# debarghabhattofficial/yolo_tracking

Hardware: AMD Instinct MI355X
Metric: tracker.update() calls/sec @ 1024 tracks×1024 dets; 1/2/4/8 MI355X (higher is better)
Workload: dtype f64; 1 GPU; bytetrack 1024x1024, 2048 streams/GPU, inputs resident in HBM; tracker=bytetrack, tracks=1024, dets=1024, streams_per_gpu=2048, queues_per_gpu=2, parallelism=stream-sharded x1, preroll=35

## Files before the change

include/yolo_tracking_amd.h:

```cpp
#ifndef YOLO_TRACKING_AMD_H
#define YOLO_TRACKING_AMD_H

#include <stdint.h>

#ifdef __cplusplus
extern "C" {
#endif

#define YTA_OK 0
#define YTA_ERR_INVALID (-1)
#define YTA_ERR_HIP (-2)
#define YTA_ERR_CAPACITY (-3)
#define YTA_ERR_NOMEM (-4)

int yta_version(void);
const char *yta_last_error(void);
int yta_device_count(int *count);

#define YTA_AFF_IOU 0
#define YTA_AFF_GIOU 1
#define YTA_AFF_DIOU 2
#define YTA_AFF_CIOU 3
#define YTA_AFF_CENTROID 4
int yta_box_affinity(int device, int kind, const double *a, int na, const double *b, int nb,
                     double img_w, double img_h, double *out);
int yta_iou_distance(int device, const double *a, int na, const double *b, int nb,
                     const double *scores, double *out);

int yta_grid_pairs(int device, const double *a, int na, const double *b, int nb, double thresh,
                   int *pairs, int cap, int *n_pairs);

int yta_kf_xyah_initiate(int device, int n, const double *meas, double *mean, double *cov);
int yta_affine_apply(int device, int kind, int n, const double *warps, double *mean, double *cov);
int yta_kf_xyah_predict(int device, int n, double *mean, double *cov);
int yta_kf_xyah_update(int device, int n, double *mean, double *cov, const double *z);

int yta_selftest(int device);

int yta_apply_block_map(int gx, int n_streams, int *stream, int *block);

int yta_lap_limited(int device, int nr, int nc, const double *cost, double cost_limit, int *x,
                    int *y);

int yta_lap_padded(int device, int nr, int nc, const double *cost, int *x, int *y);

int yta_lap_rect(int device, int nr, int nc, const double *cost, int *x, int *y);
int yta_lap_first_round(int device, int na, int nb, const double *cost, int *rx, int *done,
                        int *n_tight);

typedef struct yta_bytetrack yta_bytetrack;
typedef struct {
    double track_thresh;
    double match_thresh;
    int track_buffer;
    int frame_rate;
} yta_bytetrack_params;

int yta_bytetrack_create(int device, int n_streams, int track_capacity, int max_dets,
                         const yta_bytetrack_params *params, yta_bytetrack **engine);
int yta_bytetrack_destroy(yta_bytetrack *engine);
int yta_bytetrack_reset(yta_bytetrack *engine);

int yta_bytetrack_reserve(yta_bytetrack *engine, int track_capacity, int max_dets);
int yta_bytetrack_capacity(yta_bytetrack *engine, int *track_capacity, int *max_dets);

int yta_bytetrack_update(yta_bytetrack *engine, const double *dets, const int *det_offsets,
                         long long *next_id, double *out, int out_capacity, int *out_offsets);

int yta_bytetrack_update_device(yta_bytetrack *engine, const double *d_dets,
                                const int *d_det_offsets, double *d_out, int *d_out_counts);
int yta_bytetrack_sync(yta_bytetrack *engine);
int yta_bytetrack_next_ids(yta_bytetrack *engine, long long *next_id);

int yta_bytetrack_submit(yta_bytetrack *engine, const double *dets, const int *det_offsets,
                         const long long *next_id, double *out, int out_capacity);
int yta_bytetrack_collect(yta_bytetrack *engine, long long *next_id, int *out_offsets);
int yta_bytetrack_pipe_stats(yta_bytetrack *engine, double *stats, int n, int reset);
int yta_bytetrack_submit_f32(yta_bytetrack *engine, const float *dets, const int *det_offsets,
                             const long long *next_id, double *out, int out_capacity);
int yta_bytetrack_update_f32(yta_bytetrack *engine, const float *dets, const int *det_offsets,
                             long long *next_id, double *out, int out_capacity,
                             int *out_offsets);

int yta_bytetrack_update_streams(yta_bytetrack *engine, int n_streams, const int *stream_ids,
                                 const double *dets, const int *det_offsets, long long *next_id,
                                 double *out, int out_capacity, int *out_offsets);
int yta_bytetrack_update_device_masked(yta_bytetrack *engine, const int *d_active,
                                       const double *d_dets, const int *d_det_offsets,
                                       double *d_out, int *d_out_counts);
int yta_bytetrack_reset_stream(yta_bytetrack *engine, int stream);

int yta_bytetrack_get_state(yta_bytetrack *engine, int stream, int *n_tracks, long long *ints,
// ... 314 lines not shown
```

yolo_tracking_amd/_lib.py:

```python
import ctypes
import os

import numpy as np

_HERE = os.path.dirname(os.path.abspath(__file__))
LIB_PATH = os.environ.get("YTA_LIBRARY") or os.path.join(_HERE, "libyta.so")


class PwArgs(ctypes.Structure):
    _fields_ = [("x1", ctypes.c_void_p), ("x1n", ctypes.c_longlong), ("x1c", ctypes.c_longlong),
                ("x1p", ctypes.c_longlong), ("x2", ctypes.c_void_p), ("x2n", ctypes.c_longlong),
                ("x2c", ctypes.c_longlong), ("x2p", ctypes.c_longlong), ("w", ctypes.c_void_p),
                ("bias", ctypes.c_void_p), ("res", ctypes.c_void_p), ("rn", ctypes.c_longlong),
                ("rc", ctypes.c_longlong), ("rp", ctypes.c_longlong), ("y", ctypes.c_void_p),
                ("yn", ctypes.c_longlong), ("yc", ctypes.c_longlong), ("yp", ctypes.c_longlong),
                ("k1", ctypes.c_int), ("k2", ctypes.c_int), ("G", ctypes.c_int),
                ("cout_g", ctypes.c_int), ("P", ctypes.c_int), ("N", ctypes.c_int),
                ("relu", ctypes.c_int), ("pad", ctypes.c_int)]


YTA_OK = 0
YTA_ERR_INVALID = -1
YTA_ERR_HIP = -2
YTA_ERR_CAPACITY = -3
# ... 68 lines not shown
    "yta_device_count": ([_P], _I),
    "yta_box_affinity": ([_I, _I, _P, _I, _P, _I, _D, _D, _P], _I),
    "yta_iou_distance": ([_I, _P, _I, _P, _I, _P, _P], _I),
    "yta_kf_xyah_initiate": ([_I, _I, _P, _P, _P], _I),
    "yta_kf_xyah_predict": ([_I, _I, _P, _P], _I),
    "yta_kf_xyah_update": ([_I, _I, _P, _P, _P], _I),
    "yta_grid_pairs": ([_I, _P, _I, _P, _I, _D, _P, _I, _P], _I),
    "yta_lap_limited": ([_I, _I, _I, _P, _D, _P, _P], _I),
    "yta_lap_padded": ([_I, _I, _I, _P, _P, _P], _I),
    "yta_lap_rect": ([_I, _I, _I, _P, _P, _P], _I),
    "yta_lap_first_round": ([_I, _I, _I, _P, _P, _P, _P], _I),
    "yta_affine_apply": ([_I, _I, _I, _P, _P, _P], _I),
    "yta_bytetrack_create": ([_I, _I, _I, _I, _P, _P], _I),
    "yta_bytetrack_destroy": ([_P], _I),
    "yta_bytetrack_reset": ([_P], _I),
    "yta_bytetrack_reserve": ([_P, _I, _I], _I),
    "yta_bytetrack_capacity": ([_P, _P, _P], _I),
    "yta_bytetrack_update": ([_P, _P, _P, _P, _P, _I, _P], _I),
    "yta_bytetrack_update_device": ([_P, _P, _P, _P, _P], _I),
    "yta_bytetrack_sync": ([_P], _I),
    "yta_bytetrack_update_streams": ([_P, _I, _P, _P, _P, _P, _P, _I, _P], _I),
    "yta_bytetrack_update_device_masked": ([_P, _P, _P, _P, _P, _P], _I),
    "yta_bytetrack_reset_stream": ([_P, _I], _I),
    "yta_bytetrack_submit": ([_P, _P, _P, _P, _P, _I], _I),
    "yta_bytetrack_collect": ([_P, _P, _P], _I),
    "yta_bytetrack_pipe_stats": ([_P, _P, _I, _I], _I),
    "yta_bytetrack_next_ids": ([_P, _P], _I),
    "yta_bytetrack_submit_f32": ([_P, _P, _P, _P, _P, _I], _I),
    "yta_bytetrack_update_f32": ([_P, _P, _P, _P, _P, _I, _P], _I),
    "yta_bytetrack_get_state": ([_P, _I, _P, _P, _P, _P], _I),
    "yta_bytetrack_profile": ([_P, _I], _I),
    "yta_bytetrack_profile_collect": ([_P, _P, _P], _I),
    "yta_bytetrack_stats": ([_P, _P], _I),
    "yta_bytetrack_modes": ([_P, _P, _I], _I),
    "yta_bytetrack_hip_stream": ([_P, _P], _I),
    "yta_bytetrack_set_lds": ([_P, _I], _I),
    "yta_bytetrack_update_tensors": ([_P, _P, _P, _I, _LL, _P, _P, _P, _P, _LL, _P, _P], _I),
    "yta_bytetrack_tensor_stats": ([_P, _P, _I], _I),
    "yta_botsort_update_tensors": ([_P, _P, _P, _I, _LL, _P, _P, _LL, _P, _P, _P, _P, _LL, _P, _P],
                                   _I),
    "yta_ocsort_update_tensors": ([_P, _P, _P, _I, _LL, _P, _P, _P, _P, _P, _LL, _P, _P], _I),
    "yta_ocsort_tensor_stats": ([_P, _P, _I], _I),
    "yta_ocsort_next_ids": ([_P, _P], _I),
    "yta_deepocsort_update_tensors": ([_P, _P, _P, _I, _LL, _P, _P, _LL, _P, _P, _P, _P, _P, _LL,
                                       _P, _P], _I),
    "yta_deepocsort_tensor_stats": ([_P, _P, _I], _I),
    "yta_deepocsort_next_ids": ([_P, _P], _I),
    "yta_hybridsort_update_tensors": ([_P, _P, _P, _I, _LL, _P, _P, _LL, _P, _P, _P, _LL, _P, _P],
                                      _I),
    "yta_hybridsort_tensor_stats": ([_P, _P, _I], _I),
    "yta_hybridsort_next_ids": ([_P, _P], _I),
    "yta_selftest": ([_I], _I),
    "yta_apply_block_map": ([_I, _I, _P, _P], _I),
    "yta_botsort_create": ([_I, _I, _I, _I, _I, _P, _P], _I),
    "yta_botsort_update": ([_P, _P, _P, _P, _P, _P, _P, _I, _P], _I),
    "yta_botsort_update_device": ([_P, _P, _P, _P, _P, _P, _P], _I),
    "yta_botsort_get_features": ([_P, _I, _P, _P, _P, _P], _I),
    "yta_botsort_update_streams": ([_P, _I, _P, _P, _P, _P, _P, _P, _P, _I, _P], _I),
    "yta_ocsort_create": ([_I, _I, _I, _I, _P, _P], _I),
    "yta_ocsort_destroy": ([_P], _I),
    "yta_ocsort_reset": ([_P], _I),
    "yta_ocsort_capacity": ([_P, _P, _P], _I),
    "yta_ocsort_update": ([_P, _P, _P, _P, _P, _P, _I, _P], _I),
    "yta_ocsort_update_device": ([_P, _P, _P, _P, _P, _P], _I),
    "yta_ocsort_update_streams": ([_P, _I, _P, _P, _P, _P, _P, _P, _I, _P], _I),
    "yta_ocsort_update_device_masked": ([_P, _P, _P, _P, _P, _P, _P], _I),
    "yta_ocsort_reset_stream": ([_P, _I], _I),
    "yta_ocsort_sync": ([_P], _I),
    "yta_ocsort_get_state": ([_P, _I, _P, _P, _P, _P], _I),
    "yta_ocsort_stats": ([_P, _P], _I),
    "yta_ocsort_lap_stats": ([_P, _P, _I], _I),
    "yta_ocsort_hip_stream": ([_P, _P], _I),
    "yta_kf7_run": ([_I, _I, _I, _P, _P, _P, _P], _I),
    "yta_deepocsort_create": ([_I, _I, _I, _I, _I, _P, _P], _I),
    "yta_deepocsort_destroy": ([_P], _I),
    "yta_deepocsort_reset": ([_P], _I),
    "yta_deepocsort_capacity": ([_P, _P, _P], _I),
    "yta_deepocsort_update": ([_P, _P, _P, _P, _P, _P, _P, _P, _I, _P], _I),
    "yta_deepocsort_update_device": ([_P, _P, _P, _P, _P, _P, _P, _P], _I),
    "yta_deepocsort_update_streams": ([_P, _I, _P, _P, _P, _P, _P, _P, _P, _P, _I, _P], _I),
    "yta_deepocsort_update_device_masked": ([_P, _P, _P, _P, _P, _P, _P, _P, _P], _I),
    "yta_deepocsort_reset_stream": ([_P, _I], _I),
    "yta_deepocsort_sync": ([_P], _I),
    "yta_deepocsort_get_state": ([_P, _I, _P, _P, _P, _P, _P], _I),
    "yta_deepocsort_stats": ([_P, _P], _I),
    "yta_deepocsort_lap_stats": ([_P, _P, _I], _I),
    "yta_deepocsort_hip_stream": ([_P, _P], _I),
    "yta_kf8_run": ([_I, _I, _I, _P, _P, _P, _P, _P], _I),
    "yta_hybridsort_create": ([_I, _I, _I, _I, _I, _P, _P], _I),
    "yta_hybridsort_destroy": ([_P], _I),
    "yta_hybridsort_reset": ([_P], _I),
    "yta_hybridsort_capacity": ([_P, _P, _P], _I),
    "yta_hybridsort_update": ([_P, _P, _P, _P, _P, _P, _I, _P], _I),
    "yta_hybridsort_update_device": ([_P, _P, _P, _P, _P, _P], _I),
    "yta_hybridsort_update_streams": ([_P, _I, _P, _P, _P, _P, _P, _P, _I, _P], _I),
    "yta_hybridsort_update_device_masked": ([_P, _P, _P, _P, _P, _P, _P], _I),
    "yta_hybridsort_reset_stream": ([_P, _I], _I),
    "yta_hybridsort_sync": ([_P], _I),
    "yta_hybridsort_get_state": ([_P, _I, _P, _P, _P, _P, _P, _P], _I),
    "yta_hybridsort_classes": ([_P, _I, _P, _I, _P], _I),
    "yta_hybridsort_stats": ([_P, _P], _I),
    "yta_hybridsort_lap_stats": ([_P, _P, _I], _I),
    "yta_hybridsort_hip_stream": ([_P, _P], _I),
    "yta_kf9_run": ([_I, _I, _I, _P, _P, _P, _P], _I),
    "yta_gsi_interpolate": ([_I, _P, _I, _I, _I, _I, _P, ctypes.c_longlong, _P], _I),
    "yta_gsi_smooth": ([_I, _P, _P, _P, _P, _P, _I, _P], _I),
# ... 255 lines not shown
```

yolo_tracking_amd/csrc/bytetrack.hip:

```cpp
#include <chrono>
#include <algorithm>
#include <cmath>
#include <cstring>
#include <memory>
#include <new>
#include <thread>
#include <vector>

#include "bytetrack.hpp"
#include "host_pool.hpp"
#include "oc_host.hpp"

namespace yta {
namespace {

#ifndef YTA_BLK1
#define YTA_BLK1 1024
#endif
#ifndef YTA_BLK23
#define YTA_BLK23 256
#endif
#ifndef YTA_BLKF
#define YTA_BLKF 256
#endif
// ... 586 lines not shown
        const bool give = nd <= 2 * nt && 5LL * 8 * nh <= hand_cap;
        handed = give;
#pragma unroll
        for (int h = 0; h < 2; ++h) {
            const int e = h ? t0 + e1 : e0;
            if (cat[h] == 1) {
                const int p = n_high + (e & 0xFFFF);
                a.high[db + p] = h ? i1 : i0;
                a.high_box[db + p] = b[h];
                a.high_score[db + p] = r[h].v[4];
                if (give) {
                    hand[p] = b[h].x1;
                    hand[nh + p] = b[h].y1;
                    hand[2 * nh + p] = b[h].x2;
                    hand[3 * nh + p] = b[h].y2;
                    hand[4 * nh + p] = r[h].v[4];
                }
            } else if (cat[h] == 2) {
                const int p = n_second + (e >> 16);
                a.second[db + p] = h ? i1 : i0;
                a.second_box[db + p] = b[h];
            }
        }
        n_high += nh;
        n_second += ns;
    }
    s1_frame_counters(a.cnt + s, nd, n_high, n_second);
    return n_high;
}

template <typename F>
__device__ __forceinline__ void s1_row_edges(const BtArgs &a, int s, const GridView &gv,
                                             const GridHdr &h, const Box &rb, F f) {
    const long long db = (long long)s * a.MAXD;
    const double thresh = a.match_thresh;
    auto scored = [&](int j, const Box &cb, double w) {
        const double dist = 1 - iou(rb, cb);
        const double cost = 1 - (1 - dist) * w;
        if (cost < thresh) f(j, cost);
    };
    grid_query(gv, h, rb, scored, [&](int j) {
        const Box cb = a.high_box[db + j];
        if (intersects(rb, cb)) scored(j, cb, a.high_score[db + j]);
    });
}

__device__ __forceinline__ GridView s1_grid_hbm(const BtArgs &a, int s) {
    const long long db = (long long)s * a.MAXD;
    return GridView{a.g_hdr + s, a.g_cell + (long long)s * (GRID_MAX_CELLS + 1), a.g_ids + db,
                    a.g_boxes + db, a.g_w + db, a.g_big + db};
}

__host__ __device__ inline long long s1_grid_bytes(long long C) {
    return 4 * (GRID_MAX_CELLS + 1) + C * (4 + 32 + 8 + 4) + 5 * 16;
}

template <typename HBox, typename HW>
__device__ __forceinline__ void s1_edges_body(const BtArgs &a, int s, int nc, int nr,
                                              const GridView &gv, HBox hbox, HW hw,
                                              GridScratch &gs, int *wsum, int &spill, int *cdeg,
                                              int &n_edges, int (&rn)[4], int (&rc)[4]) {
    const int t = threadIdx.x, nt = blockDim.x;
    const long long tb = (long long)s * a.CAP, SC = (long long)a.S * a.CAP;
    grid_build(nc, hbox, hw, gv, gs, wsum);
    const GridHdr h = gs.hdr;
    YTA_STAMP(1);
    for (int base = t; base < nr; base += 4 * nt) {
        Box rb[4];
#pragma unroll
        for (int b = 0; b < 4; ++b)
            if (base + b * nt < nr) rb[b] = a.pool_box[tb + base + b * nt];
#pragma unroll
        for (int b = 0; b < 4; ++b) {
            const int i = base + b * nt;
            if (i >= nr) continue;
            int n = 0, first = -1;
            s1_row_edges(a, s, gv, h, rb[b], [&](int j, double cost) {
                if (n == 0) first = j;
                if (n < E_SLOTS) {
                    a.e_col[n * SC + tb + i] = j;
                    a.e_cost[n * SC + tb + i] = cost;
                }
                ++n;
                atomicAdd(cdeg + j, 1);
            });
            a.e_cnt[tb + i] = n;
            if (n > E_SLOTS) spill = 1;
            if (n) atomicAdd(&n_edges, n);
            if (base == t) {
                rn[b] = n;
                rc[b] = n == 1 ? first : -1;
            }
        }
    }
}

constexpr int WQ_CAP = 384;
__device__ __forceinline__ Box s1_box(const GridView &gv, int k) {
    const double *x = gv.sx;
    const int n = gv.sn;
    return Box{x[k], x[n + k], x[2 * n + k], x[3 * n + k]};
}
struct EdgeWaveQ {
    unsigned q[WQ_CAP];
    int cnt[WAVE];
    int first[WAVE];
};

__device__ __forceinline__ double bperm_f64(double v, int src_lane) {
    const long long b = __double_as_longlong(v);
    const int lo = __builtin_amdgcn_ds_bpermute(src_lane << 2, (int)b);
    const int hi = __builtin_amdgcn_ds_bpermute(src_lane << 2, (int)(b >> 32));
    return __longlong_as_double(((long long)hi << 32) | (unsigned)lo);
}

__device__ __forceinline__ void s1_edges_rows_wave(const BtArgs &a, int s, int nr,
                                                   const GridView &gv, const GridHdr &h,
                                                   EdgeWaveQ &wq, int &spill, int *cdeg,
                                                   int &n_edges, int (&rn)[4], int (&rc)[4]) {
    const int t = threadIdx.x, nt = blockDim.x, lane = lane_id();
    const long long tb = (long long)s * a.CAP, db = (long long)s * a.MAXD;
    const long long SC = (long long)a.S * a.CAP;
    const double thresh = a.match_thresh;
    int m = 0;
    for (int base = t - lane; base < nr; base += nt, ++m) {
        const int i = base + lane;
        const bool on = i < nr;
        Box rb{0.0, 0.0, 0.0, 0.0};
        if (on) rb = a.pool_box[tb + i];
        int cx0 = 0, cx1 = -1, cy0 = 0, cy1 = -1;
        if (!on || !grid_scan_window(h, rb, cx0, cx1, cy0, cy1)) cy1 = cy0 - 1;
        int cnt = 0;
        for (int cy = cy0; cy <= cy1; ++cy)
            cnt += gv.cell_start[cy * h.gx + cx1 + 1] - gv.cell_start[cy * h.gx + cx0];
        const int incl = wave_inclusive_scan(cnt);
        const int off = incl - cnt;
        const int total = __builtin_amdgcn_readlane(incl, WAVE - 1);
        wq.cnt[lane] = 0;
        wq.first[lane] = -1;
        for (int lo = 0; lo < total; lo += WQ_CAP) {
            const int hi = lo + WQ_CAP;
            if (off < hi && off + cnt > lo) {
                int idx = off;
                for (int cy = cy0; cy <= cy1 && idx < hi; ++cy) {
                    const int b = gv.cell_start[cy * h.gx + cx0], e = gv.cell_start[cy * h.gx + cx1 + 1];
                    const int k0 = idx < lo ? lo - idx : 0;
                    const int k1 = idx + (e - b) < hi ? e - b : hi - idx;
                    for (int k = k0; k < k1; ++k) wq.q[idx + k - lo] = ((unsigned)lane << 24) | (unsigned)(b + k);
                    idx += e - b;
                }
            }
            __builtin_amdgcn_wave_barrier();
            asm volatile("s_waitcnt lgkmcnt(0)" ::: "memory");
            const int n = total - lo < WQ_CAP ? total - lo : WQ_CAP;
            int ns = 0;
            const unsigned long long lt = (1ull << lane) - 1ull;
            for (int k0 = 0; k0 < n; k0 += 2 * WAVE) {
                const int ka = k0 + lane, kb = ka + WAVE;
                const unsigned ea = wq.q[ka < n ? ka : 0], eb = wq.q[kb < n ? kb : 0];
                const int ra = (int)(ea >> 24), pa = (int)(ea & 0xFFFFFFu);
                const int rb_ = (int)(eb >> 24), pb = (int)(eb & 0xFFFFFFu);
                const Box A{bperm_f64(rb.x1, ra), bperm_f64(rb.y1, ra), bperm_f64(rb.x2, ra),
                            bperm_f64(rb.y2, ra)};
                const Box B{bperm_f64(rb.x1, rb_), bperm_f64(rb.y1, rb_), bperm_f64(rb.x2, rb_),
                            bperm_f64(rb.y2, rb_)};
                const Box ca = s1_box(gv, pa), cb = s1_box(gv, pb);
                const bool ha = (ka < n) & (A.x2 > ca.x1) & (ca.x2 > A.x1) & (A.y2 > ca.y1) &
                                (ca.y2 > A.y1);
                const bool hb = (kb < n) & (B.x2 > cb.x1) & (cb.x2 > B.x1) & (B.y2 > cb.y1) &
                                (cb.y2 > B.y1);
                const unsigned long long ba = __ballot(ha), bb = __ballot(hb);
                const int na = __popcll(ba);
                if (ha) wq.q[ns + __popcll(ba & lt)] = ea;
                if (hb) wq.q[ns + na + __popcll(bb & lt)] = eb;
                ns += na + __popcll(bb);
            }
            __builtin_amdgcn_wave_barrier();
            asm volatile("s_waitcnt lgkmcnt(0)" ::: "memory");
            for (int k0 = 0; k0 < ns; k0 += WAVE) {
                const int k = k0 + lane;
                const unsigned ent = wq.q[k < ns ? k : 0];
                const int r = (int)(ent >> 24), pos = (int)(ent & 0xFFFFFFu);
                const Box cb = s1_box(gv, pos);
                const double wj = gv.w[pos];
                const int j = gv.ids[pos];
                const Box tb_{bperm_f64(rb.x1, r), bperm_f64(rb.y1, r), bperm_f64(rb.x2, r),
                              bperm_f64(rb.y2, r)};
                if (k >= ns) continue;
                const double dist = 1 - iou(tb_, cb);
                const double cost = 1 - (1 - dist) * wj;
                if (!(cost < thresh)) continue;
                const int c = atomicAdd(&wq.cnt[r], 1);
                if (c < E_SLOTS) {
                    a.e_col[c * SC + tb + base + r] = j;
                    a.e_cost[c * SC + tb + base + r] = cost;
                }
                if (c == 0) wq.first[r] = j;
                atomicAdd(cdeg + j, 1);
            }
            __builtin_amdgcn_wave_barrier();
            asm volatile("s_waitcnt lgkmcnt(0)" ::: "memory");
        }
        int nn = wq.cnt[lane];
        int first = wq.first[lane];
        if (on)
            for (int k = 0; k < h.n_big; ++k) {
                const int j = gv.big[k];
                const Box cb = a.high_box[db + j];
                if (!intersects(rb, cb)) continue;
                const double dist = 1 - iou(rb, cb);
                const double cost = 1 - (1 - dist) * a.high_score[db + j];
                if (!(cost < thresh)) continue;
                if (nn < E_SLOTS) {
                    a.e_col[nn * SC + tb + i] = j;
                    a.e_cost[nn * SC + tb + i] = cost;
                }
                if (nn == 0) first = j;
                ++nn;
                atomicAdd(cdeg + j, 1);
            }
        if (on) {
            a.e_cnt[tb + i] = nn;
            if (nn > E_SLOTS) spill = 1;
            if (nn) atomicAdd(&n_edges, nn);
            if (m < 4) {
                rn[m] = nn;
                rc[m] = nn == 1 ? first : -1;
            }
        }
        __builtin_amdgcn_wave_barrier();
    }
}

__device__ __forceinline__ void s1_single_edges(const BtArgs &a, int s, int nc, int nr, int *cdeg,
                                                bool lds, const int (&rn)[4], const int (&rc)[4]) {
    const int t = threadIdx.x, nt = blockDim.x;
    const long long tb = (long long)s * a.CAP, db = (long long)s * a.MAXD;
    if (lds) lds_sync();
    else block_sync();
    auto row = [&](int i, int n, int c) {
        int x = -1;
        if (n == 1 && ald(cdeg + c) == 1) {
            x = c;
            cdeg[c] = ~i;
            a.e_cnt[tb + i] = 0;
        }
        a.x1[tb + i] = x;
    };
#pragma unroll
    for (int b = 0; b < 4; ++b)
        if (t + b * nt < nr) row(t + b * nt, rn[b], rc[b]);
    for (int i = t + 4 * nt; i < nr; i += nt) {
        const int n = a.e_cnt[tb + i];
        row(i, n, n == 1 ? a.e_col[tb + i] : -1);
    }
    if (lds) lds_sync();
    else block_sync();
    for (int j = t; j < nc; j += nt) {
        const int d = ald(cdeg + j);
        a.y1[db + j] = d < 0 ? ~d : -1;
    }
}

template <int NT>
__global__ __launch_bounds__(NT, NT == BLKE ? 4 : 1) void k_s1_edges(BtArgs a) {
    extern __shared__ __attribute__((aligned(16))) unsigned char smem[];
    __shared__ GridScratch gs;
    __shared__ int wsum[32];
    __shared__ int spill, n_edges;
    __shared__ EdgeWaveQ ewq[NT / WAVE];
    const int s = blockIdx.x, t = threadIdx.x, nt = blockDim.x;
    if (stream_skipped(a, s)) return;
    YTA_STAMP_BASE(66);
    YTA_STAMP(0);
    YTA_BLK(1, 0);
    BtCounters *c = a.cnt + s;
    const long long db = (long long)s * a.MAXD;
    if (t == 0) {
        spill = 0;
        n_edges = 0;
    }
    Box hb0{0.0, 0.0, 0.0, 0.0}, hb1{0.0, 0.0, 0.0, 0.0};
    double hw0 = 0.0, hw1 = 0.0;
    double *hand = reinterpret_cast<double *>(smem);
    bool handed;
    const int nc = s1_dets_fused(a, s, wsum, hand, (long long)a.lds_bytes_e, handed);
    const int nr = c->n_pool;
    YTA_STAMP(3);
    if (handed) {
        lds_sync();
        if (t < nc) {
            hb0 = Box{hand[t], hand[nc + t], hand[2 * nc + t], hand[3 * nc + t]};
            hw0 = hand[4 * nc + t];
        }
        if (t + nt < nc) {
            hb1 = Box{hand[t + nt], hand[nc + t + nt], hand[2 * nc + t + nt], hand[3 * nc + t + nt]};
            hw1 = hand[4 * nc + t + nt];
        }
        lds_sync();
    } else {
        block_sync();
        if (t < nc) {
            hb0 = a.high_box[db + t];
            hw0 = a.high_score[db + t];
        }
        if (t + nt < nc) {
            hb1 = a.high_box[db + t + nt];
            hw1 = a.high_score[db + t + nt];
        }
    }
    int rn[4] = {0, 0, 0, 0}, rc[4] = {-1, -1, -1, -1};
    if (nc > 2 * nt || s1_grid_bytes(nc) + 4LL * nc > (long long)a.lds_bytes_e) {
        int *cdeg = a.g_deg + db;
        for (int j = t; j < nc; j += nt) cdeg[j] = 0;
        block_sync();
        s1_edges_body(
            a, s, nc, nr, s1_grid_hbm(a, s), [&](int j) { return a.high_box[db + j]; },
            [&](int j) { return a.high_score[db + j]; }, gs, wsum, spill, cdeg, n_edges, rn, rc);
        s1_single_edges(a, s, nc, nr, cdeg, false, rn, rc);
        if (t == 0) c->n_edges[0] = n_edges;
        YTA_BLK(1, 1);
        return;
    }
    auto hbox = [&](int j) { return j == t ? hb0 : hb1; };
    auto hw = [&](int j) { return j == t ? hw0 : hw1; };
    Arena ar(smem, a.lds_bytes_e);
    GridView gv;
    gv.hdr = nullptr;
    gv.cell_start = ar.alloc<int>(grid_cells_for(nc) + 1);
    gv.ids = ar.alloc<int>(nc);
    gv.boxes = nullptr;
    gv.sx = ar.alloc<double>(4LL * nc);
    gv.sn = nc;
    gv.w = ar.alloc<double>(nc);
    gv.big = ar.alloc<int>(nc);
    int *cdeg = ar.alloc<int>(nc);
    for (int j = t; j < nc; j += nt) cdeg[j] = 0;
    grid_build(nc, hbox, hw, gv, gs, wsum);
    YTA_STAMP(1);
    s1_edges_rows_wave(a, s, nr, gv, gs.hdr, ewq[t / WAVE], spill, cdeg, n_edges, rn, rc);
    s1_single_edges(a, s, nc, nr, cdeg, true, rn, rc);
    if (t == 0) c->n_edges[0] = n_edges;
    YTA_STAMP(2);
    YTA_BLK(1, 1);
    if (!spill) return;
    const GridHdr h = gs.hdr;
    const GridView gg = s1_grid_hbm(a, s);
    const int ncell = h.gx * h.gy;
    if (t == 0) *gg.hdr = h;
    for (int q = t; q <= ncell; q += nt) gg.cell_start[q] = gv.cell_start[q];
    for (int q = t; q < h.n_binned; q += nt) {
        gg.ids[q] = gv.ids[q];
        gg.boxes[q] = s1_box(gv, q);
        gg.w[q] = gv.w[q];
    }
    for (int q = t; q < h.n_big; q += nt) gg.big[q] = gv.big[q];
}

__host__ __device__ inline long long s1_lap_arena_bytes(long long R, long long C, long long E) {
    return 4 * (R + 1) + 8 * R + 8 * ((C + 31) / 32 + 1) + 12 * C + 12 * E + 4 * (R + C) * 3 +
           4 * 6 * (R + C + 1) + 16 * 16 + 512;
}

__device__ __forceinline__ bool s1_lap_body(const BtArgs &a, int s, Arena &ar, LapShared &lsh) {
    const int t = threadIdx.x, nt = blockDim.x;
    BtCounters *c = a.cnt + s;
    const long long db = (long long)s * a.MAXD, tb = (long long)s * a.CAP;
    const long long SC = (long long)a.S * a.CAP;
    const int nr = c->n_pool, nc = c->n_high;
    YTA_STAMP_BASE(90);
    YTA_STAMP(0);
    int *X = a.x1 + tb;
    int *Y = a.y1 + db;
    int myr = 0, mye = 0;
    for (int i = t; i < nr; i += nt) {
        const int n = a.e_cnt[tb + i];
        myr += n > 0;
        mye += n;
    }
    int R, E;
    block_exclusive_scan<false>(myr, lsh.wsum, &R);
    block_exclusive_scan<false>(mye, lsh.wsum, &E);
    if (E == 0) {
        if (t == 0) c->n_res1 = 0;
        return true;
    }
    const int words = (nc + 31) >> 5;
    int *rid = ar.alloc_top<int>(R);
    int *row_off = ar.alloc_top<int>(R + 1);
    unsigned *cbits = ar.alloc_top<unsigned>(words);
    int *cpre = ar.alloc_top<int>(words + 1);
    int *csr_col = ar.alloc_top<int>(E);
    double *csr_cost = ar.alloc_top<double>(E);
    if (ar.fail) return false;
    for (int w = t; w < words; w += nt) cbits[w] = 0u;
    int runR = 0, runE = 0;
    for (int base = 0; base < nr; base += 8 * nt) {
        const int m = nr - base < 8 * nt ? nr - base : 8 * nt;
        const int per = (m + nt - 1) / nt;
        const int lo = base + t * per;
        const int hi = lo + per < base + m ? lo + per : base + m;
        int cnt[8], mr = 0, me = 0;
#pragma unroll
        for (int k = 0; k < 8; ++k) {
            cnt[k] = lo + k < hi ? a.e_cnt[tb + lo + k] : 0;
            mr += cnt[k] > 0;
            me += cnt[k];
        }
        int totR, totE;
// ... 1488 lines not shown
    int pipe_head = 0, pipe_count = 0;
    hipStream_t s_in = nullptr, s_out = nullptr;
    double pstat[24] = {};
    bool prof = false;
    bool graphs = true;
    hipGraph_t g_graph = nullptr;
    hipGraphExec_t g_exec = nullptr;
    BtArgs g_args{};
    const void *g_ptrs[5] = {};
    long long g_cap = -1;
    long long g_captures = 0, g_replays = 0;
    std::vector<hipEvent_t> ev;
    size_t ev_used = 0;
    std::unique_ptr<CopyPool> pool;
    struct TSlot {
        hipEvent_t in = nullptr, done = nullptr;
        int *h_counts = nullptr, *m_counts = nullptr;
        long long *h_nid = nullptr, *m_nid = nullptr;
        int2 *h_live = nullptr, *m_live = nullptr;
        std::vector<long long> cum_at;
        long long seq = -1, gen = -1;
    };
    std::vector<TSlot *> t_ring;
    std::vector<long long> t_cum;
    std::vector<long long> t_base_live, t_base_cum;
    bool t_dirty = false;
    long long t_seq = 0, t_gen = 0;
    double *t_det = nullptr;
    long long t_det_cap = 0;
    int *t_off = nullptr;
    float *t_feat = nullptr;
    long long t_feat_cap = 0;
    std::vector<void *> t_retired;
    long long tstat[4] = {};
};

namespace {

constexpr int BT_PHASES = 6;
#ifndef YTA_LDS1_KB
#define YTA_LDS1_KB 150
#endif
constexpr size_t BT_LDS_BYTES = YTA_LDS1_KB * 1024;
constexpr size_t BT_LDS23_BYTES = 32 * 1024;
#ifndef YTA_LDSF_KB
#define YTA_LDSF_KB 32
#endif
constexpr size_t BT_LDSF_BYTES = YTA_LDSF_KB * 1024;
#ifndef YTA_LDSL_KB
#define YTA_LDSL_KB 38
#endif
constexpr size_t BT_LDSL_BYTES = YTA_LDSL_KB * 1024;
#ifndef YTA_LDSE_KB
#define YTA_LDSE_KB 62
#endif
constexpr size_t BT_LDSE_BYTES = YTA_LDSE_KB * 1024;

#ifndef YTA_STAGE_THREADS
#define YTA_STAGE_THREADS 8
#endif
#ifndef YTA_STAGE_CHUNKS
#define YTA_STAGE_CHUNKS 4
#endif
void par_copy(yta_bytetrack *e, void *dst, const void *src, size_t bytes) {
    constexpr size_t MIN_PIECE = 2u << 20;
    const unsigned hw = std::thread::hardware_concurrency();
    const size_t T = std::min<size_t>(std::min<unsigned>(hw ? hw : 1, YTA_STAGE_THREADS),
                                      bytes / MIN_PIECE);
    if (T <= 1) {
        memcpy(dst, src, bytes);
        return;
    }
    if (!e->pool) e->pool.reset(new CopyPool(std::min<unsigned>(hw, YTA_STAGE_THREADS) - 1));
    e->pool->copy(dst, src, bytes, (int)T);
}
constexpr int STAGE_CHUNKS = YTA_STAGE_CHUNKS;

bool host_pinned(const void *p, size_t bytes, void **dev = nullptr) {
    if (dev) *dev = nullptr;
    if (!p || !bytes) return false;
    hipPointerAttribute_t at;
    if (hipPointerGetAttributes(&at, p) != hipSuccess) {
        (void)hipGetLastError();
        return false;
    }
    if (at.type != hipMemoryTypeHost) return false;
    hipDeviceptr_t base = nullptr;
    size_t size = 0;
    if (hipPointerGetAttribute(&base, HIP_POINTER_ATTRIBUTE_RANGE_START_ADDR,
                               (hipDeviceptr_t)p) != hipSuccess ||
        hipPointerGetAttribute(&size, HIP_POINTER_ATTRIBUTE_RANGE_SIZE, (hipDeviceptr_t)p) !=
            hipSuccess) {
        (void)hipGetLastError();
        return false;
    }
    const char *b = (const char *)base, *q = (const char *)p;
    const bool inside = b && q >= b && bytes <= size && (size_t)(q - b) <= size - bytes;
    if (inside && dev) *dev = at.devicePointer;
    return inside;
}
inline size_t stage_chunk(size_t bytes) {
    const int n = bytes >= (16u << 20) ? STAGE_CHUNKS : 1;
    return ((bytes + n - 1) / n + 63) & ~(size_t)63;
}
int stage_h2d(yta_bytetrack *e, void *dev, void *pinned, const void *src, size_t bytes,
              hipStream_t st) {
    const size_t ch = stage_chunk(bytes);
// ... 1775 lines not shown
```

yolo_tracking_amd/csrc/grid.hpp:

```cpp
#pragma once
#include "common.hpp"
#include "geometry.hpp"
#include "lap.hpp"

namespace yta {

constexpr int GRID_MAX_CELLS = 2048;

__host__ __device__ __forceinline__ int grid_cells_for(int n) {
    const int c = 2 * n + 16;
    return c < GRID_MAX_CELLS ? c : GRID_MAX_CELLS;
}

struct GridHdr {
    double ox, oy, inv_g, maxw, maxh, g;
    int gx, gy, n_big, n_binned;
};

struct GridView {
    GridHdr *hdr;
    int *cell_start;
    int *ids;
    Box *boxes;
    double *w;
    int *big;
    const Box *by_id = nullptr;
    double *sx = nullptr;
    int sn = 0;
};

__device__ __forceinline__ Box grid_box(const GridView &gv, int k) {
    if (gv.sx) return Box{gv.sx[k], gv.sx[gv.sn + k], gv.sx[2 * gv.sn + k], gv.sx[3 * gv.sn + k]};
    return gv.boxes ? gv.boxes[k] : gv.by_id[gv.ids[k]];
}


__host__ __device__ __forceinline__ bool box_usable(const Box &b) {
    const double w = b.x2 - b.x1, h = b.y2 - b.y1;
    return w > 0.0 && h > 0.0 && isfinite(b.x1) && isfinite(b.y1) && isfinite(b.x2) &&
           isfinite(b.y2) && isfinite(w) && isfinite(h);
}

__device__ __forceinline__ int grid_cell_1d(double x, double o, double inv_g, int n) {
    double f = floor((x - o) * inv_g);
    f = f < 0.0 ? 0.0 : (f > (double)(n - 1) ? (double)(n - 1) : f);
    return (int)f;
}

struct GridScratch {
    double red[8 * 16];
    GridHdr hdr;
    unsigned long long maxw_bits, maxh_bits;
};

__device__ __forceinline__ void block_reduce6(double v[6], const int op[6], double *red) {
    const int wv = threadIdx.x / WAVE, nw = blockDim.x / WAVE, lane = lane_id();
    for (int k = 0; k < 6; ++k) v[k] = wave_reduce(op[k], v[k]);
    if (lane == 0)
        for (int k = 0; k < 6; ++k) red[8 * wv + k] = v[k];
    block_sync();
    for (int k = 0; k < 6; ++k)
        v[k] = wave_reduce(op[k], lane < nw ? red[8 * lane + k] : red_ident(op[k]));
    __syncthreads();
}

template <typename BoxOf, typename WOf>
__device__ __forceinline__ void grid_build(int n, BoxOf box, WOf wof, GridView gv, GridScratch &gs,
                                           int *wsum) {
    const int t = threadIdx.x, nt = blockDim.x;
    YTA_STAMP_ABS(110);
    double v[6] = {0.0, 0.0, INFINITY, INFINITY, -INFINITY, -INFINITY};
    const int ops[6] = {RED_SUM, RED_SUM, RED_MIN, RED_MIN, RED_MAX, RED_MAX};
    for (int i = t; i < n; i += nt) {
        const Box b = box(i);
        if (!box_usable(b)) continue;
        v[0] += fmax(b.x2 - b.x1, b.y2 - b.y1);
        v[1] += 1.0;
        v[2] = fmin(v[2], b.x1);
        v[3] = fmin(v[3], b.y1);
        v[4] = fmax(v[4], b.x1);
        v[5] = fmax(v[5], b.y1);
    }
    if (t == 0) {
        gs.maxw_bits = 0ull;
        gs.maxh_bits = 0ull;
        gs.hdr.n_big = 0;
    }
    block_reduce6(v, ops, gs.red);
    YTA_STAMP_ABS(111);
    const double mean = v[1] > 0 ? v[0] / v[1] : 1.0;
    const double bthr = 4.0 * mean;
    auto binned = [&](const Box &b) {
        return box_usable(b) && !(b.x2 - b.x1 > bthr) && !(b.y2 - b.y1 > bthr);
    };
    GridHdr h;
    if (!(v[4] >= v[2])) {
        h.ox = h.oy = 0.0;
        h.g = 1.0;
        h.inv_g = 1.0;
        h.gx = h.gy = 1;
    } else {
        double g = mean;
        const double ex = v[4] - v[2], ey = v[5] - v[3];
        double gxf = floor(ex / g) + 1.0, gyf = floor(ey / g) + 1.0;
        const double max_cells = (double)grid_cells_for(n);
        while (gxf * gyf > max_cells) {
            g *= 1.25;
            gxf = floor(ex / g) + 1.0;
            gyf = floor(ey / g) + 1.0;
        }
        h.ox = v[2];
        h.oy = v[3];
        h.g = g;
        h.inv_g = 1.0 / g;
        h.gx = (int)gxf;
        h.gy = (int)gyf;
    }
    const int ncell = h.gx * h.gy;
    int *cs = gv.cell_start;
    for (int c = t; c <= ncell; c += nt) cs[c] = 0;
    block_sync();
    YTA_STAMP_ABS(112);
    auto cell_of = [&](const Box &b) {
        return grid_cell_1d(b.y1, h.oy, h.inv_g, h.gy) * h.gx + grid_cell_1d(b.x1, h.ox, h.inv_g, h.gx);
    };
    double mw = 0.0, mh = 0.0;
    for (int i = t; i < n; i += nt) {
        const Box b = box(i);
        if (!box_usable(b)) continue;
        if (!binned(b)) {
            gv.big[atomicAdd(&gs.hdr.n_big, 1)] = i;
            continue;
        }
        mw = fmax(mw, b.x2 - b.x1);
        mh = fmax(mh, b.y2 - b.y1);
        atomicAdd(&cs[cell_of(b) + 1], 1);
    }
    mw = wave_reduce(RED_MAX, mw);
    mh = wave_reduce(RED_MAX, mh);
    if (lane_id() == 0) {
        atomicMax(&gs.maxw_bits, (unsigned long long)__double_as_longlong(mw));
        atomicMax(&gs.maxh_bits, (unsigned long long)__double_as_longlong(mh));
    }
    block_sync();
    YTA_STAMP_ABS(113);
    {
        const int per = (ncell + nt - 1) / nt;
        const int c0 = t * per, c1 = c0 + per < ncell ? c0 + per : ncell;
        int mine = 0;
        for (int c = c0; c < c1; ++c) mine += ald(cs + c + 1);
        int tot;
        int run = block_exclusive_scan(mine, wsum, &tot);
        for (int c = c0; c < c1; ++c) {
            const int k = ald(cs + c + 1);
            cs[c + 1] = run;
            run += k;
        }
        if (t == 0) {
            h.n_big = gs.hdr.n_big;
            h.n_binned = tot;
            h.maxw = __longlong_as_double((long long)gs.maxw_bits);
            h.maxh = __longlong_as_double((long long)gs.maxh_bits);
            gs.hdr = h;
            if (gv.hdr) *gv.hdr = h;
        }
    }
    block_sync();
    YTA_STAMP_ABS(115);
    for (int i = t; i < n; i += nt) {
        const Box b = box(i);
        if (!binned(b)) continue;
        const int pos = atomicAdd(&cs[cell_of(b) + 1], 1);
        gv.ids[pos] = i;
        if (gv.boxes) gv.boxes[pos] = b;
        if (gv.sx) {
            gv.sx[pos] = b.x1;
            gv.sx[gv.sn + pos] = b.y1;
            gv.sx[2 * gv.sn + pos] = b.x2;
            gv.sx[3 * gv.sn + pos] = b.y2;
        }
        if (gv.w) gv.w[pos] = wof(i);
    }
    block_sync();
    YTA_STAMP_ABS(116);
}

template <typename Hit>
__device__ __forceinline__ void grid_scan(const GridView &gv, const GridHdr &h, const Box &T,
                                          Hit hit) {
    if (h.n_binned == 0) return;
    if (!(T.x2 > T.x1 && T.y2 > T.y1)) return;
    const double lx = (T.x1 - h.maxw * (1.0 + 1e-12)) - (fabs(T.x1) + h.maxw) * 1e-12;
    const double ly = (T.y1 - h.maxh * (1.0 + 1e-12)) - (fabs(T.y1) + h.maxh) * 1e-12;
    const double fx1 = floor((T.x2 - h.ox) * h.inv_g), fy1 = floor((T.y2 - h.oy) * h.inv_g);
    if (fx1 < 0.0 || fy1 < 0.0) return;
    const int cx0 = grid_cell_1d(lx, h.ox, h.inv_g, h.gx);
    const int cy0 = grid_cell_1d(ly, h.oy, h.inv_g, h.gy);
    const int cx1 = fx1 > (double)(h.gx - 1) ? h.gx - 1 : (int)fx1;
    const int cy1 = fy1 > (double)(h.gy - 1) ? h.gy - 1 : (int)fy1;
    auto wt = [&](int k) { return gv.w ? gv.w[k] : 1.0; };
    int b = ald(gv.cell_start + cy0 * h.gx + cx0), e = ald(gv.cell_start + cy0 * h.gx + cx1 + 1);
    for (int cy = cy0; cy <= cy1; ++cy) {
        int nb = 0, ne = 0;
        if (cy < cy1) {
            const int base = (cy + 1) * h.gx;
            nb = ald(gv.cell_start + base + cx0);
            ne = ald(gv.cell_start + base + cx1 + 1);
        }
        int k = b;
        for (; k + 1 < e; k += 2) {
            const Box b0 = grid_box(gv, k), b1 = grid_box(gv, k + 1);
            const int i0 = gv.ids[k], i1 = gv.ids[k + 1];
            const double w0 = wt(k), w1 = wt(k + 1);
            if (intersects(T, b0)) hit(k, i0, b0, w0);
            if (intersects(T, b1)) hit(k + 1, i1, b1, w1);
        }
        if (k < e) {
            const Box b0 = grid_box(gv, k);
            if (intersects(T, b0)) hit(k, gv.ids[k], b0, wt(k));
        }
        b = nb;
        e = ne;
    }
}

__device__ __forceinline__ bool grid_scan_window(const GridHdr &h, const Box &T, int &cx0, int &cx1,
                                                 int &cy0, int &cy1) {
// ... 133 lines not shown
```

yolo_tracking_amd/csrc/util.hip:

```cpp
#include <cstdarg>
#include <cstdio>

#include "common.hpp"

namespace yta {

static thread_local char g_err[512] = "";

void set_error(const char *fmt, ...) {
    va_list ap;
    va_start(ap, fmt);
    vsnprintf(g_err, sizeof(g_err), fmt, ap);
    va_end(ap);
}

int select_device(int device) {
    int n = 0;
    hipError_t e = hipGetDeviceCount(&n);
    if (e != hipSuccess || n == 0) {
        set_error("no HIP device available (%s)", e == hipSuccess ? "0 devices" : hipGetErrorString(e));
        return YTA_ERR_HIP;
    }
    if (device < 0 || device >= n) {
        set_error("device %d out of range (%d devices)", device, n);
        return YTA_ERR_INVALID;
    }
    YTA_HIP(hipSetDevice(device));
    return YTA_OK;
}

hipError_t host_wait(hipStream_t s) {
    constexpr int MAX_DEV = 64;
    thread_local hipEvent_t ev[MAX_DEV] = {};
    int dev = 0;
    hipError_t e = hipGetDevice(&dev);
    if (e != hipSuccess) return e;
    if (s) {
        hipDevice_t sd;
        if (hipStreamGetDevice(s, &sd) == hipSuccess) dev = (int)sd;
    }
    if (dev < 0 || dev >= MAX_DEV) return hipStreamSynchronize(s);
    if (!ev[dev]) {
        int cur = -1;
        (void)hipGetDevice(&cur);
        if (cur != dev) (void)hipSetDevice(dev);
        e = hipEventCreateWithFlags(&ev[dev], hipEventBlockingSync | hipEventDisableTiming);
        if (cur != dev) (void)hipSetDevice(cur);
        if (e != hipSuccess) {
            ev[dev] = nullptr;
            return hipStreamSynchronize(s);
        }
    }
    e = hipEventRecord(ev[dev], s);
    if (e != hipSuccess) return e;
    return hipEventSynchronize(ev[dev]);
}

}

extern "C" {

int yta_version(void) { return 1; }

const char *yta_last_error(void) { return yta::g_err; }

int yta_device_count(int *count) {
    YTA_CHECK(count, YTA_ERR_INVALID, "null count");
    int n = 0;
    hipError_t e = hipGetDeviceCount(&n);
    *count = e == hipSuccess ? n : 0;
    return YTA_OK;
}

int yta_apply_block_map(int gx, int n_streams, int *stream, int *block) {
    YTA_CHECK(gx > 0 && n_streams > 0 && stream && block, YTA_ERR_INVALID, "bad block map shape");
    for (int lin = 0; lin < gx * n_streams; ++lin)
        yta::xcd_stream_blocks(lin, gx, n_streams, stream[lin], block[lin]);
    return YTA_OK;
}

}
```

Before: 2.274 million calls/s.

## Use 16-bit packed box coordinates and 16-bit ids in stage-1 grid pre-filter

The stage-1 edge pre-filter now compares conservatively rounded 16-bit quantized boxes, packed into a uint2 and checked with a packed u16 max, instead of exchanging four f64 coordinates per candidate across lanes. Candidates that pass are checked again exactly in f64 before the IoU is computed. Work-queue entries, grid ids and the big-box list move to 16-bit storage in LDS, with big ids stored at the tail of ids16, and the queue capacity is doubled. This cuts LDS footprint and cross-lane permutes. In exchange, grids with more than 1024 columns fall back to the HBM path, and a host-side pretest helper is added for validation.

Measured after the change: 2.314 million calls/s (median of 6 runs). 1.02x the previous value.

```diff
diff --git a/include/yolo_tracking_amd.h b/include/yolo_tracking_amd.h
--- a/include/yolo_tracking_amd.h
+++ b/include/yolo_tracking_amd.h
@@ -38,6 +38,9 @@
 int yta_selftest(int device);
 
 int yta_apply_block_map(int gx, int n_streams, int *stream, int *block);
+
+int yta_s1_pretest(int nr, const double *pool, int nc, const double *high, const double *score,
+                   double thresh, unsigned char *out);
 
 int yta_lap_limited(int device, int nr, int nc, const double *cost, double cost_limit, int *x,
                     int *y);
diff --git a/yolo_tracking_amd/_lib.py b/yolo_tracking_amd/_lib.py
--- a/yolo_tracking_amd/_lib.py
+++ b/yolo_tracking_amd/_lib.py
@@ -144,6 +144,7 @@
     "yta_hybridsort_next_ids": ([_P, _P], _I),
     "yta_selftest": ([_I], _I),
     "yta_apply_block_map": ([_I, _I, _P, _P], _I),
+    "yta_s1_pretest": ([_I, _P, _I, _P, _P, _D, _P], _I),
     "yta_botsort_create": ([_I, _I, _I, _I, _I, _P, _P], _I),
     "yta_botsort_update": ([_P, _P, _P, _P, _P, _P, _P, _I, _P], _I),
     "yta_botsort_update_device": ([_P, _P, _P, _P, _P, _P, _P], _I),
diff --git a/yolo_tracking_amd/csrc/bytetrack.hip b/yolo_tracking_amd/csrc/bytetrack.hip
--- a/yolo_tracking_amd/csrc/bytetrack.hip
+++ b/yolo_tracking_amd/csrc/bytetrack.hip
@@ -662,7 +662,7 @@
 }
 
 __host__ __device__ inline long long s1_grid_bytes(long long C) {
-    return 4 * (GRID_MAX_CELLS + 1) + C * (4 + 32 + 8 + 4) + 5 * 16;
+    return 4 * (GRID_MAX_CELLS + 1) + C * (2 + 32 + 8 + 8) + 5 * 16;
 }
 
 template <typename HBox, typename HW>
@@ -705,16 +705,17 @@
     }
 }
 
-constexpr int WQ_CAP = 384;
+constexpr int WQ_CAP = 768;
+constexpr int WQ_POS_BITS = 10;
 __device__ __forceinline__ Box s1_box(const GridView &gv, int k) {
     const double *x = gv.sx;
     const int n = gv.sn;
     return Box{x[k], x[n + k], x[2 * n + k], x[3 * n + k]};
 }
 struct EdgeWaveQ {
-    unsigned q[WQ_CAP];
+    unsigned short q[WQ_CAP];
     int cnt[WAVE];
-    int first[WAVE];
+    unsigned short first[WAVE];
 };
 
 __device__ __forceinline__ double bperm_f64(double v, int src_lane) {
@@ -722,6 +723,11 @@
     const int lo = __builtin_amdgcn_ds_bpermute(src_lane << 2, (int)b);
     const int hi = __builtin_amdgcn_ds_bpermute(src_lane << 2, (int)(b >> 32));
     return __longlong_as_double(((long long)hi << 32) | (unsigned)lo);
+}
+
+__device__ __forceinline__ uint2 bperm_u2(const uint2 &v, int src_lane) {
+    return make_uint2((unsigned)__builtin_amdgcn_ds_bpermute(src_lane << 2, (int)v.x),
+                      (unsigned)__builtin_amdgcn_ds_bpermute(src_lane << 2, (int)v.y));
 }
 
 __device__ __forceinline__ void s1_edges_rows_wave(const BtArgs &a, int s, int nr,
@@ -732,6 +738,9 @@
     const long long tb = (long long)s * a.CAP, db = (long long)s * a.MAXD;
     const long long SC = (long long)a.S * a.CAP;
     const double thresh = a.match_thresh;
+    constexpr unsigned WQ_POS_MASK = (1u << WQ_POS_BITS) - 1u;
+    const double psc = grid_pack_scale(h);
+    const int nc = gv.sn;
     int m = 0;
     for (int base = t - lane; base < nr; base += nt, ++m) {
         const int i = base + lane;
@@ -740,6 +749,7 @@
         if (on) rb = a.pool_box[tb + i];
         int cx0 = 0, cx1 = -1, cy0 = 0, cy1 = -1;
         if (!on || !grid_scan_window(h, rb, cx0, cx1, cy0, cy1)) cy1 = cy0 - 1;
+        const uint2 rp = box_pack16(rb, h.ox, h.oy, psc);
         int cnt = 0;
         for (int cy = cy0; cy <= cy1; ++cy)
             cnt += gv.cell_start[cy * h.gx + cx1 + 1] - gv.cell_start[cy * h.gx + cx0];
@@ -747,7 +757,7 @@
         const int off = incl - cnt;
         const int total = __builtin_amdgcn_readlane(incl, WAVE - 1);
         wq.cnt[lane] = 0;
-        wq.first[lane] = -1;
+        wq.first[lane] = 0xFFFF;
         for (int lo = 0; lo < total; lo += WQ_CAP) {
             const int hi = lo + WQ_CAP;
             if (off < hi && off + cnt > lo) {
@@ -756,7 +766,8 @@
                     const int b = gv.cell_start[cy * h.gx + cx0], e = gv.cell_start[cy * h.gx + cx1 + 1];
                     const int k0 = idx < lo ? lo - idx : 0;
                     const int k1 = idx + (e - b) < hi ? e - b : hi - idx;
-                    for (int k = k0; k < k1; ++k) wq.q[idx + k - lo] = ((unsigned)lane << 24) | (unsigned)(b + k);
+                    for (int k = k0; k < k1; ++k)
+                        wq.q[idx + k - lo] = (unsigned short)((lane << WQ_POS_BITS) | (b + k));
                     idx += e - b;
                 }
             }
@@ -768,21 +779,16 @@
             for (int k0 = 0; k0 < n; k0 += 2 * WAVE) {
                 const int ka = k0 + lane, kb = ka + WAVE;
                 const unsigned ea = wq.q[ka < n ? ka : 0], eb = wq.q[kb < n ? kb : 0];
-                const int ra = (int)(ea >> 24), pa = (int)(ea & 0xFFFFFFu);
-                const int rb_ = (int)(eb >> 24), pb = (int)(eb & 0xFFFFFFu);
-                const Box A{bperm_f64(rb.x1, ra), bperm_f64(rb.y1, ra), bperm_f64(rb.x2, ra),
-                            bperm_f64(rb.y2, ra)};
-                const Box B{bperm_f64(rb.x1, rb_), bperm_f64(rb.y1, rb_), bperm_f64(rb.x2, rb_),
-                            bperm_f64(rb.y2, rb_)};
-                const Box ca = s1_box(gv, pa), cb = s1_box(gv, pb);
-                const bool ha = (ka < n) & (A.x2 > ca.x1) & (ca.x2 > A.x1) & (A.y2 > ca.y1) &
-                                (ca.y2 > A.y1);
-                const bool hb = (kb < n) & (B.x2 > cb.x1) & (cb.x2 > B.x1) & (B.y2 > cb.y1) &
-                                (cb.y2 > B.y1);
+                const int ra = (int)(ea >> WQ_POS_BITS), pa = (int)(ea & WQ_POS_MASK);
+                const int rb_ = (int)(eb >> WQ_POS_BITS), pb = (int)(eb & WQ_POS_MASK);
+                const uint2 A = bperm_u2(rp, ra), B = bperm_u2(rp, rb_);
+                const uint2 ca = gv.pk[pa], cb = gv.pk[pb];
+                const bool ha = (ka < n) & box16_meet(A, ca);
+                const bool hb = (kb < n) & box16_meet(B, cb);
                 const unsigned long long ba = __ballot(ha), bb = __ballot(hb);
                 const int na = __popcll(ba);
-                if (ha) wq.q[ns + __popcll(ba & lt)] = ea;
-                if (hb) wq.q[ns + na + __popcll(bb & lt)] = eb;
+                if (ha) wq.q[ns + __popcll(ba & lt)] = (unsigned short)ea;
+                if (hb) wq.q[ns + na + __popcll(bb & lt)] = (unsigned short)eb;
                 ns += na + __popcll(bb);
             }
             __builtin_amdgcn_wave_barrier();
@@ -790,13 +796,15 @@
             for (int k0 = 0; k0 < ns; k0 += WAVE) {
                 const int k = k0 + lane;
                 const unsigned ent = wq.q[k < ns ? k : 0];
-                const int r = (int)(ent >> 24), pos = (int)(ent & 0xFFFFFFu);
+                const int r = (int)(ent >> WQ_POS_BITS), pos = (int)(ent & WQ_POS_MASK);
                 const Box cb = s1_box(gv, pos);
                 const double wj = gv.w[pos];
-                const int j = gv.ids[pos];
+                const int j = gv.ids16[pos];
                 const Box tb_{bperm_f64(rb.x1, r), bperm_f64(rb.y1, r), bperm_f64(rb.x2, r),
                               bperm_f64(rb.y2, r)};
                 if (k >= ns) continue;
+                if (!((tb_.x2 > cb.x1) & (cb.x2 > tb_.x1) & (tb_.y2 > cb.y1) & (cb.y2 > tb_.y1)))
+                    continue;
                 const double dist = 1 - iou(tb_, cb);
                 const double cost = 1 - (1 - dist) * wj;
                 if (!(cost < thresh)) continue;
@@ -805,7 +813,7 @@
                     a.e_col[c * SC + tb + base + r] = j;
                     a.e_cost[c * SC + tb + base + r] = cost;
                 }
-                if (c == 0) wq.first[r] = j;
+                if (c == 0) wq.first[r] = (unsigned short)j;
                 atomicAdd(cdeg + j, 1);
             }
             __builtin_amdgcn_wave_barrier();
@@ -815,7 +823,7 @@
         int first = wq.first[lane];
         if (on)
             for (int k = 0; k < h.n_big; ++k) {
-                const int j = gv.big[k];
+                const int j = gv.ids16[nc - 1 - k];
                 const Box cb = a.high_box[db + j];
                 if (!intersects(rb, cb)) continue;
                 const double dist = 1 - iou(rb, cb);
@@ -920,7 +928,8 @@
         }
     }
     int rn[4] = {0, 0, 0, 0}, rc[4] = {-1, -1, -1, -1};
-    if (nc > 2 * nt || s1_grid_bytes(nc) + 4LL * nc > (long long)a.lds_bytes_e) {
+    if (nc > 2 * nt || nc > (1 << WQ_POS_BITS) ||
+        s1_grid_bytes(nc) + 4LL * nc > (long long)a.lds_bytes_e) {
         int *cdeg = a.g_deg + db;
         for (int j = t; j < nc; j += nt) cdeg[j] = 0;
         block_sync();
@@ -938,12 +947,14 @@
     GridView gv;
     gv.hdr = nullptr;
     gv.cell_start = ar.alloc<int>(grid_cells_for(nc) + 1);
-    gv.ids = ar.alloc<int>(nc);
+    gv.ids = nullptr;
+    gv.big = nullptr;
+    gv.ids16 = ar.alloc<unsigned short>(nc);
     gv.boxes = nullptr;
     gv.sx = ar.alloc<double>(4LL * nc);
     gv.sn = nc;
     gv.w = ar.alloc<double>(nc);
-    gv.big = ar.alloc<int>(nc);
+    gv.pk = ar.alloc<uint2>(nc);
     int *cdeg = ar.alloc<int>(nc);
     for (int j = t; j < nc; j += nt) cdeg[j] = 0;
     grid_build(nc, hbox, hw, gv, gs, wsum);
@@ -960,11 +971,11 @@
     if (t == 0) *gg.hdr = h;
     for (int q = t; q <= ncell; q += nt) gg.cell_start[q] = gv.cell_start[q];
     for (int q = t; q < h.n_binned; q += nt) {
-        gg.ids[q] = gv.ids[q];
+        gg.ids[q] = gv.ids16[q];
         gg.boxes[q] = s1_box(gv, q);
         gg.w[q] = gv.w[q];
     }
-    for (int q = t; q < h.n_big; q += nt) gg.big[q] = gv.big[q];
+    for (int q = t; q < h.n_big; q += nt) gg.big[q] = gv.ids16[nc - 1 - q];
 }
 
 __host__ __device__ inline long long s1_lap_arena_bytes(long long R, long long C, long long E) {
@@ -2559,7 +2570,7 @@
 #endif
 constexpr size_t BT_LDSL_BYTES = YTA_LDSL_KB * 1024;
 #ifndef YTA_LDSE_KB
-#define YTA_LDSE_KB 62
+#define YTA_LDSE_KB 63
 #endif
 constexpr size_t BT_LDSE_BYTES = YTA_LDSE_KB * 1024;
 
diff --git a/yolo_tracking_amd/csrc/grid.hpp b/yolo_tracking_amd/csrc/grid.hpp
--- a/yolo_tracking_amd/csrc/grid.hpp
+++ b/yolo_tracking_amd/csrc/grid.hpp
@@ -27,7 +27,39 @@
     const Box *by_id = nullptr;
     double *sx = nullptr;
     int sn = 0;
+    unsigned short *ids16 = nullptr;
+    uint2 *pk = nullptr;
 };
+
+__host__ __device__ __forceinline__ unsigned pack16_dn(double x, double o, double sc) {
+    const double v = floor((x - o) * sc);
+    return v >= 0.0 ? (v < 65535.0 ? (unsigned)v : 65535u) : 0u;
+}
+__host__ __device__ __forceinline__ unsigned pack16_up(double x, double o, double sc) {
+    const double v = ceil((x - o) * sc);
+    return v <= 65535.0 ? (v > 0.0 ? (unsigned)v : 0u) : 65535u;
+}
+__host__ __device__ __forceinline__ uint2 box_pack16(const Box &b, double ox, double oy,
+                                                     double sc) {
+    uint2 p;
+    p.x = pack16_dn(b.x1, ox, sc) | (pack16_dn(b.y1, oy, sc) << 16);
+    p.y = pack16_up(b.x2, ox, sc) | (pack16_up(b.y2, oy, sc) << 16);
+    return p;
+}
+__host__ __device__ __forceinline__ double grid_pack_scale(const GridHdr &h) {
+    const double rx = (double)h.gx * h.g + h.maxw, ry = (double)h.gy * h.g + h.maxh;
+    const double r = rx > ry ? rx : ry;
+    return r > 0.0 && r < INFINITY ? 65534.0 / r : 0.0;
+}
+typedef unsigned short u16x2 __attribute__((ext_vector_type(2)));
+__host__ __device__ __forceinline__ bool pk16_ge(unsigned u, unsigned v) {
+    const u16x2 m = __builtin_elementwise_max(__builtin_bit_cast(u16x2, u),
+                                              __builtin_bit_cast(u16x2, v));
+    return __builtin_bit_cast(unsigned, m) == u;
+}
+__host__ __device__ __forceinline__ bool box16_meet(const uint2 &a, const uint2 &b) {
+    return (int)pk16_ge(a.y, b.x) & (int)pk16_ge(b.y, a.x);
+}
 
 __device__ __forceinline__ Box grid_box(const GridView &gv, int k) {
     if (gv.sx) return Box{gv.sx[k], gv.sx[gv.sn + k], gv.sx[2 * gv.sn + k], gv.sx[3 * gv.sn + k]};
@@ -39,6 +71,41 @@
     const double w = b.x2 - b.x1, h = b.y2 - b.y1;
     return w > 0.0 && h > 0.0 && isfinite(b.x1) && isfinite(b.y1) && isfinite(b.x2) &&
            isfinite(b.y2) && isfinite(w) && isfinite(h);
+}
+
+__host__ __device__ __forceinline__ double grid_mean_size(const double v[6]) {
+    return v[1] > 0 ? v[0] / v[1] : 1.0;
+}
+__host__ __device__ __forceinline__ bool grid_binned(const Box &b, double bthr) {
+    return box_usable(b) && !(b.x2 - b.x1 > bthr) && !(b.y2 - b.y1 > bthr);
+}
+__host__ __device__ __forceinline__ GridHdr grid_geometry(const double v[6], int n) {
+    GridHdr h;
+    h.maxw = h.maxh = 0.0;
+    h.n_big = h.n_binned = 0;
+    if (!(v[4] >= v[2])) {
+        h.ox = h.oy = 0.0;
+        h.g = 1.0;
+        h.inv_g = 1.0;
+        h.gx = h.gy = 1;
+        return h;
+    }
+    double g = grid_mean_size(v);
+    const double ex = v[4] - v[2], ey = v[5] - v[3];
+    double gxf = floor(ex / g) + 1.0, gyf = floor(ey / g) + 1.0;
+    const double max_cells = (double)grid_cells_for(n);
+    while (gxf * gyf > max_cells) {
+        g *= 1.25;
+        gxf = floor(ex / g) + 1.0;
+        gyf = floor(ey / g) + 1.0;
+    }
+    h.ox = v[2];
+    h.oy = v[3];
+    h.g = g;
+    h.inv_g = 1.0 / g;
+    h.gx = (int)gxf;
+    h.gy = (int)gyf;
+    return h;
 }
 
 __device__ __forceinline__ int grid_cell_1d(double x, double o, double inv_g, int n) {
@@ -88,34 +155,9 @@
     }
     block_reduce6(v, ops, gs.red);
     YTA_STAMP_ABS(111);
-    const double mean = v[1] > 0 ? v[0] / v[1] : 1.0;
-    const double bthr = 4.0 * mean;
-    auto binned = [&](const Box &b) {
-        return box_usable(b) && !(b.x2 - b.x1 > bthr) && !(b.y2 - b.y1 > bthr);
-    };
-    GridHdr h;
-    if (!(v[4] >= v[2])) {
-        h.ox = h.oy = 0.0;
-        h.g = 1.0;
-        h.inv_g = 1.0;
-        h.gx = h.gy = 1;
-    } else {
-        double g = mean;
-        const double ex = v[4] - v[2], ey = v[5] - v[3];
-        double gxf = floor(ex / g) + 1.0, gyf = floor(ey / g) + 1.0;
-        const double max_cells = (double)grid_cells_for(n);
-        while (gxf * gyf > max_cells) {
-            g *= 1.25;
-            gxf = floor(ex / g) + 1.0;
-            gyf = floor(ey / g) + 1.0;
-        }
-        h.ox = v[2];
-        h.oy = v[3];
-        h.g = g;
-        h.inv_g = 1.0 / g;
-        h.gx = (int)gxf;
-        h.gy = (int)gyf;
-    }
+    const double bthr = 4.0 * grid_mean_size(v);
+    auto binned = [&](const Box &b) { return grid_binned(b, bthr); };
+    GridHdr h = grid_geometry(v, n);
     const int ncell = h.gx * h.gy;
     int *cs = gv.cell_start;
     for (int c = t; c <= ncell; c += nt) cs[c] = 0;
@@ -129,7 +171,9 @@
         const Box b = box(i);
         if (!box_usable(b)) continue;
         if (!binned(b)) {
-            gv.big[atomicAdd(&gs.hdr.n_big, 1)] = i;
+            const int k = atomicAdd(&gs.hdr.n_big, 1);
+            if (gv.ids16) gv.ids16[gv.sn - 1 - k] = (unsigned short)i;
+            else gv.big[k] = i;
             continue;
         }
         mw = fmax(mw, b.x2 - b.x1);
@@ -167,12 +211,15 @@
     }
     block_sync();
     YTA_STAMP_ABS(115);
+    const double psc = gv.pk ? grid_pack_scale(gs.hdr) : 0.0;
     for (int i = t; i < n; i += nt) {
         const Box b = box(i);
         if (!binned(b)) continue;
         const int pos = atomicAdd(&cs[cell_of(b) + 1], 1);
-        gv.ids[pos] = i;
+        if (gv.ids16) gv.ids16[pos] = (unsigned short)i;
+        else gv.ids[pos] = i;
         if (gv.boxes) gv.boxes[pos] = b;
+        if (gv.pk) gv.pk[pos] = box_pack16(b, h.ox, h.oy, psc);
         if (gv.sx) {
             gv.sx[pos] = b.x1;
             gv.sx[gv.sn + pos] = b.y1;
diff --git a/yolo_tracking_amd/csrc/util.hip b/yolo_tracking_amd/csrc/util.hip
--- a/yolo_tracking_amd/csrc/util.hip
+++ b/yolo_tracking_amd/csrc/util.hip
@@ -1,7 +1,10 @@
+#include <math.h>
+
 #include <cstdarg>
 #include <cstdio>
 
 #include "common.hpp"
+#include "grid.hpp"
 
 namespace yta {
 
@@ -79,4 +82,50 @@
     return YTA_OK;
 }
 
+int yta_s1_pretest(int nr, const double *pool, int nc, const double *high, const double *score,
+                   double thresh, unsigned char *out) {
+    using namespace yta;
+    YTA_CHECK(nr >= 0 && nc >= 0 && nc <= 65536 && (pool || !nr) && (high || !nc) &&
+                  (score || !nc) && (out || !nr || !nc),
+              YTA_ERR_INVALID, "bad pre-test shape");
+    auto box = [](const double *p, int i) {
+        return Box{p[4 * i], p[4 * i + 1], p[4 * i + 2], p[4 * i + 3]};
+    };
+    double v[6] = {0.0, 0.0, INFINITY, INFINITY, -INFINITY, -INFINITY};
+    for (int j = 0; j < nc; ++j) {
+        const Box b = box(high, j);
+        if (!box_usable(b)) continue;
+        v[0] += fmax(b.x2 - b.x1, b.y2 - b.y1);
+        v[1] += 1.0;
+        v[2] = fmin(v[2], b.x1);
+        v[3] = fmin(v[3], b.y1);
+        v[4] = fmax(v[4], b.x1);
+        v[5] = fmax(v[5], b.y1);
+    }
+    const double bthr = 4.0 * grid_mean_size(v);
+    GridHdr h = grid_geometry(v, nc);
+    for (int j = 0; j < nc; ++j) {
+        const Box b = box(high, j);
+        if (!grid_binned(b, bthr)) continue;
+        h.maxw = fmax(h.maxw, b.x2 - b.x1);
+        h.maxh = fmax(h.maxh, b.y2 - b.y1);
+    }
+    const double sc = grid_pack_scale(h);
+    (void)score;
+    (void)thresh;
+    for (int i = 0; i < nr; ++i) {
+        const uint2 a = box_pack16(box(pool, i), h.ox, h.oy, sc);
+        for (int j = 0; j < nc; ++j) {
+            const Box b = box(high, j);
+            unsigned char r = 3;
+            if (grid_binned(b, bthr)) {
+                const uint2 c = box_pack16(b, h.ox, h.oy, sc);
+                r = box16_meet(a, c) ? 3 : 0;
+            }
+            out[(size_t)i * nc + j] = r;
+        }
+    }
+    return YTA_OK;
 }
+
+}
```
